# IONIQ6000/av1-base

Hardware: AMD Instinct MI355X
Metric: encoded frames/sec at CQ=30 (1080p intra-only) (higher is better)
Workload: dtype i32; 1 GPU; 1920x1080 60-frame all-key-frame synthclip v1 chunk per GPU, 10-bit 4:2:0, CQ=30 (base_q_idx 120), 32x32 blocks, all 13 intra candidates, 64x64 tiles, adaptive CDFs, CDEF on; frames_per_chunk=60, chunks_per_gpu=1, parallelism=chunk-per-gpu x1

## Files before the change

### av1-base_amd/csrc/av1mi_dev.h

```cpp
#ifndef AV1MI_DEV_H
#define AV1MI_DEV_H
#include <stdint.h>
#include <stddef.h>
#ifdef __HIPCC__
#define AV1MI_HD __host__ __device__
#else
#define AV1MI_HD
#endif

#define AV1MI_QM_4X4 0
#define AV1MI_QM_8X8 16
#define AV1MI_QM_16X16 80
#define AV1MI_QM_32X32 336
#define AV1MI_QM_PLANE 1360

struct Av1miQmEntry { uint32_t q, recip; };

struct Av1miDevParams {
  int width, height, bit_depth;
  int true_w, true_h;
  int mi_rows, mi_cols;
  int sb_rows, sb_cols;
  int tile_sb;
  int tile_rows, tile_cols;
  int b8_rows, b8_cols;
  int n_frames;
  int base_q_idx, qctx;
  int dc_q, ac_q;
  uint32_t dc_recip, ac_recip;
  const Av1miQmEntry *qm_tab;
  int using_qm, qm_y, qm_uv;
// ... 18 lines not shown
  int stream_cap;
  int seq_hdr_bytes, frame_hdr_bytes, inter_hdr_bytes, hdr_slot_bytes;
  int tile_size_bytes;
  int keyint, me_range;
  int subpel;
  int me_presearch;
  int lf_level[4], lf_level_inter[4], lf_sharpness;
  int enable_lr;
  int lr_code_len[4][3];
  unsigned long long lr_code_bits[4][3];
  int sgr_code_len[4][3];
  unsigned long long sgr_code_bits[4][3];
  int lr_chroma;
  int lr_code_len_uv[4][3];
  unsigned long long lr_code_bits_uv[4][3];
};

AV1MI_HD inline int av1mi_node_split(int width, int height, int min_bs_log2, int max_bs_log2, int have_mask, uint32_t mask,
                                     int sb_x, int sb_y, int ox, int oy, int bsl) {
  const int n = 1 << bsl;
  if (bsl <= 3) return 0;
  if (sb_y + oy + (n >> 1) >= height || sb_x + ox + (n >> 1) >= width) return 1;
  if (bsl <= min_bs_log2) return 0;
  if (bsl > max_bs_log2) return 1;
  if (!have_mask) return 0;
  const int bit = bsl == 6 ? 0 : (bsl == 5 ? 1 + ((oy >> 5) << 1 | (ox >> 5))
                                           : 5 + (((ox >> 4) & 1) | (((oy >> 4) & 1) << 1) | (((ox >> 5) & 1) << 2) | (((oy >> 5) & 1) << 3)));
  return (int)((mask >> bit) & 1u);
}
AV1MI_HD inline int av1mi_leaf_bsl_at(int width, int height, int min_bs_log2, int max_bs_log2, int have_mask, uint32_t mask,
// ... 3 lines not shown
    const int ox = bx & ~(n - 1), oy = by & ~(n - 1);
    if (!av1mi_node_split(width, height, min_bs_log2, max_bs_log2, have_mask, mask, sb_x, sb_y, ox, oy, bsl)) return (ox == bx && oy == by) ? bsl : 0;
  }
  return 0;
}

AV1MI_HD inline int av1mi_sext12(uint32_t v) { return (int)((v & 0xFFFu) ^ 0x800u) - 0x800; }
AV1MI_HD inline void av1mi_me_key_decode(unsigned long long key, int R, int *dy, int *dx, int *cost) {
  const int nc = 2 * R + 1, idx = (int)(key & 0xFFFF);
  *dy = idx / nc - R + 8 * av1mi_sext12((uint32_t)(key >> 52));
  *dx = idx % nc - R + 8 * av1mi_sext12((uint32_t)(key >> 40));
  *cost = (int)((key >> 16) & 0xFFFFFF);
}

AV1MI_HD inline int av1mi_frame_is_inter(const Av1miDevParams &P, int f) { return P.keyint > 1 && (f % P.keyint) != 0; }

struct Av1miBlkInfo {
  uint8_t ymode;
  uint8_t skip;
  uint8_t bsl;
  uint8_t is_inter;
  uint16_t eob[3];
  int16_t mv_row, mv_col;
  uint16_t angle;
};
static_assert(sizeof(Av1miBlkInfo) == 16, "block info is one 16-byte record");

#define AV1MI_SB_LEVELS 6144
AV1MI_HD inline int av1mi_morton8(int ux, int uy) {
  return (ux & 1) | ((uy & 1) << 1) | ((ux & 2) << 1) | ((uy & 2) << 2) | ((ux & 4) << 2) | ((uy & 4) << 3);
// ... 54 lines not shown
```

### av1-base_amd/csrc/av1mi_host.cpp

```cpp
#include <hip/hip_runtime.h>
#include <errno.h>
#include <math.h>
#include <stdarg.h>
#include <stdio.h>
#include <stdlib.h>
#include <string.h>
#include <unistd.h>

#include <algorithm>
#include <atomic>
#include <cstddef>
#include <mutex>
#include <string>
#include <thread>
#include <vector>

#include "../../include/av1mi.h"
#include "av1_tables.h"
#include "av1mi_dev.h"

extern "C" {
hipError_t av1mi_launch_partition(const Av1miDevParams *P, const void *frames, uint32_t *part, hipStream_t stream);
#define AV1MI_RECON_PROTO(name) hipError_t name(const Av1miDevParams *P, const Av1miDevParams *dP, const void *src, void *rec, int16_t *levels, \
                                               Av1miBlkInfo *blk, const void *ref, const unsigned long long *me_best, const uint32_t *part, hipStream_t s)
// ... 388 lines not shown

enum ChunkEvent { EV_START, EV_SRC_READY, EV_RECON_DONE, EV_SYM_DONE, EV_ENTROPY_DONE, EV_PACK_DONE, EV_DOWNLOAD_DONE,
                  EV_CDEF_START, EV_CDEF_DONE, EV_GROUPS_JOINED, EV_EDGE_FORK, EV_EDGE_JOIN, EV_COUNT };

struct Workspace {
  size_t cap_frames = 0;
  int scale = 0;
  Resolved res = {};
  void *d_src = nullptr, *d_rec = nullptr, *d_fin = nullptr;
  int16_t *d_levels = nullptr; Av1miBlkInfo *d_blk = nullptr;
  uint8_t *d_slots = nullptr, *d_out = nullptr, *d_hdr = nullptr;
  uint16_t *d_cdf = nullptr;
  Av1miDevParams *d_params = nullptr;
  uint32_t *d_tile_bytes = nullptr, *d_tile_off = nullptr, *d_frame_size = nullptr, *d_payload = nullptr, *d_sym = nullptr;
  uint32_t *d_streams = nullptr, *d_combos = nullptr;
  unsigned long long *d_frame_off = nullptr, *d_sse = nullptr;
  int *d_overflow = nullptr;
  unsigned long long *d_me = nullptr;
  void *d_stage = nullptr;
  void *d_cd = nullptr;
  unsigned long long *d_me_sub = nullptr;
  uint16_t *d_quarter = nullptr;
  uint32_t *d_centre = nullptr;
  uint32_t *d_part = nullptr;
  uint32_t *d_me64 = nullptr;
  Av1miQmEntry *d_qm = nullptr;
  std::vector<Av1miQmEntry> h_qm; int qm_key = -1;
  uint8_t *d_lrc = nullptr;
  unsigned long long *d_lrsse = nullptr;
  unsigned long long *d_cdef_err = nullptr;
  int8_t *d_cdef_idx = nullptr;
  uint8_t *d_cdef_sel = nullptr;
  uint8_t *h_out = nullptr;
  size_t out_cap = 0, me64_bytes = 0, h_out_cap = 0;
  std::vector<std::pair<void *, bool>> owned;
};

template <class T>
hipError_t ws_alloc(Workspace &w, T *&p, size_t bytes, bool host = false) {
  for (auto b = w.owned.begin(); p && b != w.owned.end(); ++b)
    if (b->first == (void *)p) { (void)(b->second ? hipHostFree(p) : hipFree(p)); w.owned.erase(b); break; }
  void *v = nullptr;
  const hipError_t e = host ? hipHostMalloc(&v, bytes, hipHostMallocDefault) : hipMalloc(&v, bytes);
  if (e == hipSuccess) w.owned.emplace_back(v, host);
  p = (T *)v;
  return e;
}

// ... 54 lines not shown
    free_workspace(c);
    const size_t nf = n_frames, slot = (size_t)tile_slot_bytes(r, c->cap_scale);
    for (void **b : { &w.d_src, &w.d_rec, &w.d_fin }) HIPCHK(c, ws_alloc(w, *b, nf * frame_bytes));
    HIPCHK(c, ws_alloc(w, w.d_levels, nf * nsb * AV1MI_SB_LEVELS * sizeof(int16_t)));
    HIPCHK(c, ws_alloc(w, w.d_blk, nf * nb8 * sizeof(Av1miBlkInfo)));
    HIPCHK(c, hipMemsetAsync(w.d_blk, 0, nf * nb8 * sizeof(Av1miBlkInfo), c->stream));
    HIPCHK(c, ws_alloc(w, w.d_slots, nf * ntile * slot * 2));
    w.out_cap = nf * (ntile * (slot + 4) + 256);
    HIPCHK(c, ws_alloc(w, w.d_out, w.out_cap));
    HIPCHK(c, ws_alloc(w, w.d_hdr, 256 + nf * 512));
    HIPCHK(c, ws_alloc(w, w.d_cdf, Av1miCdfLayout::TOTAL * sizeof(uint16_t)));
    HIPCHK(c, ws_alloc(w, w.d_params, sizeof(Av1miDevParams)));
    for (uint32_t **b : { &w.d_tile_bytes, &w.d_tile_off, &w.d_sym, &w.d_combos }) HIPCHK(c, ws_alloc(w, *b, nf * nsb * 4));
    HIPCHK(c, ws_alloc(w, w.d_streams, nf * ntile * (size_t)tile_stream_cap(r, c->cap_scale) * 4));
    for (uint32_t **b : { &w.d_frame_size, &w.d_payload }) HIPCHK(c, ws_alloc(w, *b, nf * 4));
    HIPCHK(c, ws_alloc(w, w.d_frame_off, (nf + 1) * 8));
    HIPCHK(c, ws_alloc(w, w.d_sse, nf * 3 * 8));
    HIPCHK(c, ws_alloc(w, w.d_overflow, 4));
    HIPCHK(c, ws_alloc(w, w.d_me, nf * nb8 * 8));
    w.cap_frames = n_frames; w.scale = c->cap_scale;
  }
  const size_t nf = w.cap_frames;
  if (r.padded && !w.d_stage) HIPCHK(c, ws_alloc(w, w.d_stage, nf * (size_t)p.width * p.height * 3 / 2 * bps));
  if (p.partition_search && !w.d_part) HIPCHK(c, ws_alloc(w, w.d_part, nf * nsb * sizeof(uint32_t)));
  if (p.me_presearch && !w.d_quarter) {
    HIPCHK(c, ws_alloc(w, w.d_quarter, nf * (size_t)(r.cw / 4) * (r.ch / 4) * sizeof(uint16_t)));
    HIPCHK(c, ws_alloc(w, w.d_centre, nf * nsb * sizeof(uint32_t)));
  }
  if (p.subpel && !w.d_me_sub) HIPCHK(c, ws_alloc(w, w.d_me_sub, nf * nb8 * 8));
  if (p.block_log2 >= 6 && p.keyint > 1) {
    const size_t nc = 2 * (size_t)(p.me_range ? p.me_range : 8) + 1, need = nf * nsb * nc * nc * sizeof(uint32_t);
    if (w.me64_bytes < need) { w.me64_bytes = 0; HIPCHK(c, ws_alloc(w, w.d_me64, need)); w.me64_bytes = need; }
  }
// ... 17 lines not shown
      for (int pt = 0; pt < 2; pt++)
        for (int l2 = 2; l2 <= 5; l2++)
          for (int i = 0; i < (1 << (2 * l2)); i++) {
            const uint32_t q = (uint32_t)(i ? r.ac_q : r.dc_q);
            const uint32_t q2 = (q * av1_qm_iwt[r.qm_level][pt][off[l2 - 2] + i] + 16) >> 5;
            w.h_qm[pt * AV1MI_QM_PLANE + off[l2 - 2] + i] = { q2, (uint32_t)((((uint64_t)1 << 32) + q2 - 1) / q2) };
          }
      HIPCHK(c, hipMemcpyAsync(w.d_qm, w.h_qm.data(), w.h_qm.size() * sizeof(Av1miQmEntry), hipMemcpyHostToDevice, c->stream));
      w.qm_key = key;
    }
  }
  return AV1MI_OK;
}

Av1miDevParams dev_params(const Resolved &r, uint32_t n_frames, int scale, const uint32_t *part, const Av1miQmEntry *qm,
                          unsigned long long *cdef_err, int8_t *cdef_idx, uint8_t *cdef_sel) {
  const av1mi_params &p = r.p;
  Av1miDevParams P;
  memset(&P, 0, sizeof(P));
  P.width = r.cw; P.height = r.ch; P.bit_depth = p.bit_depth; P.true_w = (int)p.width; P.true_h = (int)p.height;
  P.mi_rows = r.ch / 4; P.mi_cols = r.cw / 4; P.b8_rows = r.ch / 8; P.b8_cols = r.cw / 8; P.sb_rows = r.sb_rows; P.sb_cols = r.sb_cols;
  P.tile_sb = r.tile_sb; P.tile_rows = r.tile_rows; P.tile_cols = r.tile_cols;
  P.n_frames = (int)n_frames;
  P.base_q_idx = r.qidx;
  P.qctx = r.qidx <= 20 ? 0 : (r.qidx <= 60 ? 1 : (r.qidx <= 120 ? 2 : 3));
  P.dc_q = r.dc_q; P.ac_q = r.ac_q;
  P.dc_recip = (uint32_t)((((uint64_t)1 << 32) + P.dc_q - 1) / P.dc_q);
  P.ac_recip = (uint32_t)((((uint64_t)1 << 32) + P.ac_q - 1) / P.ac_q);
  P.using_qm = p.enable_qm ? 1 : 0; P.qm_y = P.qm_uv = r.qm_level;
  P.qm_tab = p.enable_qm && r.qm_level < 15 ? qm : nullptr;
  P.max_bs_log2 = (int)p.block_log2;
// ... 2 lines not shown
  P.mode_mask = p.intra_mode_mask ? (p.intra_mode_mask & 0x1FFF) : 0x0007;
  P.angle_delta = p.intra_angle_delta ? 1 : 0; P.edge_filter = p.intra_edge_filter ? 1 : 0; P.cfl = p.cfl ? 1 : 0; P.tx_search = p.tx_search ? 1 : 0;
  P.enable_cdef = p.enable_cdef ? 1 : 0;
  P.cdef_y_pri = p.cdef_y_pri; P.cdef_y_sec = p.cdef_y_sec; P.cdef_uv_pri = p.cdef_uv_pri; P.cdef_uv_sec = p.cdef_uv_sec;
  P.cdef_damping = p.cdef_damping; P.cdef_search = (int)p.cdef_search;
  if (p.cdef_search) { P.cdef_bits = (int)p.cdef_search - 1; P.cdef_err = cdef_err; P.cdef_idx = cdef_idx; P.cdef_sel = cdef_sel; }
  P.disable_cdf_update = p.cdf_update ? 0 : 1;
  P.stride_y = r.cw; P.stride_c = r.cw / 2; P.frame_samples = (long)r.cw * r.ch * 3 / 2;
  P.plane_off_u = (long)r.cw * r.ch; P.plane_off_v = P.plane_off_u + (long)(r.cw / 2) * (r.ch / 2);
  P.tile_slot_bytes = tile_slot_bytes(r, scale); P.stream_cap = tile_stream_cap(r, scale); P.tile_size_bytes = 4;
  P.keyint = (int)p.keyint; P.me_range = (int)p.me_range; P.subpel = p.subpel ? 1 : 0; P.me_presearch = p.me_presearch ? 1 : 0;
  P.hdr_slot_bytes = 512;
  for (int i = 0; i < 4; i++) { P.lf_level[i] = deblock_level(r, true); P.lf_level_inter[i] = deblock_level(r, false); }
  P.enable_lr = (int)p.enable_lr;
  P.lr_chroma = r.lr_chroma;
  for (int rf = 0; rf < 4; rf++)
    for (int k = 0; k < 3; k++) {
      const BitString b = lr_code_of(rf, k); P.lr_code_len[rf][k] = b.len; P.lr_code_bits[rf][k] = b.bits;
      const BitString g = sgr_code_of(rf, k); P.sgr_code_len[rf][k] = g.len; P.sgr_code_bits[rf][k] = g.bits;
      const BitString u = lr_code_of_uv(rf, k); P.lr_code_len_uv[rf][k] = u.len; P.lr_code_bits_uv[rf][k] = u.bits;
    }
  return P;
}

}

extern "C" {

uint32_t av1mi_abi_version(void) { return AV1MI_ABI_VERSION; }
uint32_t av1mi_struct_sizes(uint32_t *sizes, uint32_t cap) {
// ... 245 lines not shown
static int prepare_chunk(av1mi_ctx *c, const Resolved &r, const void *frames, uint32_t n_frames, int frames_on_device, const void **d_src) {
  Av1miDevParams &P = c->P; Workspace &w = c->ws; hipStream_t s = c->stream;
  size_t str_key = 0, str_inter = 0;
  std::vector<uint8_t> seq = make_sequence_header(r), fh = make_frame_header(r, nullptr, 0, false, &str_key), fhi = make_frame_header(r, nullptr, 0, true, &str_inter);
  P.cdef_str_bit[0] = (int)str_key; P.cdef_str_bit[1] = (int)str_inter;
  P.seq_hdr_bytes = (int)seq.size(); P.frame_hdr_bytes = (int)fh.size(); P.inter_hdr_bytes = (int)fhi.size();
  if (seq.size() > 256 || fh.size() > (size_t)P.hdr_slot_bytes || fhi.size() > (size_t)P.hdr_slot_bytes) { set_err(c, "internal: header larger than its slot"); return AV1MI_E_OVERFLOW; }
  std::vector<uint8_t> blob(seq.size() + (size_t)n_frames * P.hdr_slot_bytes, 0);
  memcpy(blob.data(), seq.data(), seq.size());
  for (uint32_t f = 0; f < n_frames; f++) {
    const bool inter = av1mi_frame_is_inter(P, (int)f);
    std::vector<uint8_t> &h = inter ? fhi : fh;
    if (r.p.film_grain && f) h = make_frame_header(r, nullptr, f, inter);
    memcpy(blob.data() + seq.size() + (size_t)f * P.hdr_slot_bytes, h.data(), h.size());
  }
  std::vector<uint16_t> cdf = make_cdf_blob(r.qidx);
  HIPCHK(c, hipMemcpyAsync(w.d_hdr, blob.data(), blob.size(), hipMemcpyHostToDevice, s));
  HIPCHK(c, hipMemcpyAsync(w.d_cdf, cdf.data(), cdf.size() * 2, hipMemcpyHostToDevice, s));
  HIPCHK(c, hipMemcpyAsync(w.d_params, &P, sizeof(P), hipMemcpyHostToDevice, s));
  HIPCHK(c, hipMemsetAsync(w.d_overflow, 0, 4, s));
  HIPCHK(c, hipMemsetAsync(w.d_sse, 0, (size_t)n_frames * 24, s));
  if (P.cdef_search) HIPCHK(c, hipMemsetAsync(w.d_cdef_err, 0, (size_t)n_frames * P.sb_rows * P.sb_cols * 24 * sizeof(unsigned long long), s));
  HIPCHK(c, hipEventRecord(c->ev[EV_START], s));
  const size_t bytes = (size_t)n_frames * (r.padded ? (size_t)r.p.width * r.p.height * 3 / 2 : (size_t)P.frame_samples) * (P.bit_depth > 8 ? 2 : 1);
  if (!frames_on_device) HIPCHK(c, hipMemcpyAsync(r.padded ? w.d_stage : w.d_src, frames, bytes, hipMemcpyHostToDevice, s));
  if (r.padded) HIPCHK(c, av1mi_launch_pad(frames_on_device ? frames : w.d_stage, w.d_src, (int)r.p.width, (int)r.p.height, r.cw, r.ch, P.bit_depth, (int)n_frames, 0, s));
  *d_src = frames_on_device && !r.padded ? frames : w.d_src;
  if (P.part_map) HIPCHK(c, av1mi_launch_partition(&P, *d_src, w.d_part, s));
  HIPCHK(c, hipEventRecord(c->ev[EV_SRC_READY], s));
  return AV1MI_OK;
}

static decltype(&av1mi_launch_recon_u8) recon_launcher(const Av1miDevParams &P) {
  return P.max_bs_log2 >= 6 ? (P.bit_depth == 8 ? av1mi_launch_recon64_u8 : av1mi_launch_recon64_u16)
                            : (P.bit_depth == 8 ? av1mi_launch_recon_u8 : av1mi_launch_recon_u16);
// ... 96 lines not shown
      HIPCHK(c, hipEventRecord(c->grp_ev[n_grp], s));
      HIPCHK(c, hipStreamWaitEvent(c->stream3, c->grp_ev[n_grp], 0));
      HIPCHK(c, av1mi_launch_entropy(&P, w.d_cdf, w.d_levels, w.d_blk, w.d_streams, w.d_sym, w.d_combos, w.d_slots, w.d_tile_bytes, w.d_lrc,
                                     w.d_tile_off, (int)(f + 1 - grp), (int)grp, c->stream3, nullptr, nullptr, nullptr, nullptr));
      n_grp++;
    }
  }
  if (n_grp) HIPCHK(c, hipEventRecord(c->ev[EV_GROUPS_JOINED], c->stream3));
  const int rc = entropy_code(c, n_grp * grp, n_frames);
  return rc ? rc : sse_beside_range_coder(c, src);
}

static int download_chunk(av1mi_ctx *c, const Resolved &r, uint32_t n_frames, int frames_on_device, av1mi_buf *out, uint32_t *frame_sizes,
                          void *recon, av1mi_report *report) {
  const Av1miDevParams &P = c->P; Workspace &w = c->ws; hipStream_t s = c->stream, s2 = c->stream2;
  std::vector<unsigned long long> foff(n_frames + 1);
  int overflow = 0;
  HIPCHK(c, hipMemcpyAsync(foff.data(), w.d_frame_off, (n_frames + 1) * 8, hipMemcpyDeviceToHost, s));
  HIPCHK(c, hipMemcpyAsync(&overflow, w.d_overflow, 4, hipMemcpyDeviceToHost, s));
  HIPCHK(c, hipStreamSynchronize(s));
  if (overflow) {
    (void)hipStreamSynchronize(s2);
    set_err(c, "a tile outgrew its %d-byte bitstream slot or its %d-entry symbol stream", P.tile_slot_bytes, P.stream_cap);
    return AV1MI_E_OVERFLOW;
  }
  const size_t total = (size_t)foff[n_frames];
  if (total > w.out_cap) { (void)hipStreamSynchronize(s2); set_err(c, "internal: packed size exceeds buffer"); return AV1MI_E_OVERFLOW; }
  uint8_t *host = (uint8_t *)pin_acquire(total ? total : 1);
  const bool direct = host != nullptr;
  if (!direct) {
    host = (uint8_t *)malloc(total ? total : 1);
    if (!host) { (void)hipStreamSynchronize(s2); return AV1MI_E_OOM; }
    if (w.h_out_cap < total) {
      w.h_out_cap = 0;
      if (ws_alloc(w, w.h_out, total + (total >> 2) + 4096, true) == hipSuccess) w.h_out_cap = total + (total >> 2) + 4096;
    }
  }
  uint8_t *dst = direct ? host : (w.h_out ? w.h_out : host);
  hipError_t e1 = hipMemcpyAsync(dst, w.d_out, total, hipMemcpyDeviceToHost, s);
  hipError_t e2 = hipEventRecord(c->ev[EV_DOWNLOAD_DONE], s);
  if (e2 == hipSuccess) e2 = hipStreamWaitEvent(s, c->ev[EV_CDEF_DONE], 0);
  if (e1 == hipSuccess && e2 == hipSuccess && recon) {
    const void *fin = w.d_fin;
    if (r.padded) {
      e1 = av1mi_launch_pad(w.d_fin, w.d_stage, (int)r.p.width, (int)r.p.height, r.cw, r.ch, P.bit_depth, (int)n_frames, 1, s);
      fin = w.d_stage;
    }
    const size_t bytes = (size_t)n_frames * (r.padded ? (size_t)r.p.width * r.p.height * 3 / 2 : (size_t)P.frame_samples) * (P.bit_depth > 8 ? 2 : 1);
    if (e1 == hipSuccess) e1 = hipMemcpyAsync(recon, fin, bytes, frames_on_device ? hipMemcpyDeviceToDevice : hipMemcpyDeviceToHost, s);
  }
  std::vector<unsigned long long> sse(n_frames * 3);
  std::vector<uint32_t> syms;
  if (e1 == hipSuccess) e1 = hipMemcpyAsync(sse.data(), w.d_sse, (size_t)n_frames * 24, hipMemcpyDeviceToHost, s);
  if (e1 == hipSuccess && report) {
    syms.resize((size_t)n_frames * P.tile_rows * P.tile_cols);
    e1 = hipMemcpyAsync(syms.data(), w.d_sym, syms.size() * 4, hipMemcpyDeviceToHost, s);
  }
  if (e1 == hipSuccess && e2 == hipSuccess) e1 = hipEventSynchronize(c->ev[EV_DOWNLOAD_DONE]);
  if (e1 == hipSuccess && e2 == hipSuccess && dst != host) memcpy(host, dst, total);
  if (e1 == hipSuccess) e1 = hipStreamSynchronize(s);
  if (e1 != hipSuccess || e2 != hipSuccess) {
    (void)hipStreamSynchronize(s2);
    av1mi_free(host);
    set_err(c, "device-to-host copy failed: %s", hipGetErrorString(e1 != hipSuccess ? e1 : e2));
    return AV1MI_E_HIP;
  }
  out->data = host; out->size = total;
  if (frame_sizes) for (uint32_t f = 0; f < n_frames; f++) frame_sizes[f] = (uint32_t)(foff[f + 1] - foff[f]);
  if (report) {
    memset(report, 0, sizeof(*report));
    report->frames = n_frames; report->bytes = total; report->chunks = 1;
    report->cap_scale = (uint32_t)c->cap_scale; report->gpus_used = 1u << (c->device & 31);
    const double mx = (double)((1 << P.bit_depth) - 1);
    for (int pl = 0; pl < 3; pl++) {
      double t = 0;
      for (uint32_t f = 0; f < n_frames; f++) t += (double)sse[f * 3 + pl];
      report->sse[pl] = t;
      const double npx = (double)n_frames * P.width * P.height / (pl ? 4 : 1);
      report->psnr[pl] = t > 0 ? 10.0 * log10(mx * mx * npx / t) : 99.0;
    }
    for (uint32_t v : syms) { report->n_symbols += v; if (v > report->max_tile_symbols) report->max_tile_symbols = v; }
    (void)hipEventElapsedTime(&report->ms_h2d, c->ev[EV_START], c->ev[EV_SRC_READY]);
    (void)hipEventElapsedTime(&report->ms_recon, c->ev[EV_SRC_READY], c->ev[EV_RECON_DONE]);
    (void)hipEventElapsedTime(&report->ms_cdef, c->ev[EV_CDEF_START], c->ev[EV_CDEF_DONE]);
    (void)hipEventElapsedTime(&report->ms_entropy, c->ev[EV_RECON_DONE], c->ev[EV_ENTROPY_DONE]);
    (void)hipEventElapsedTime(&report->ms_symbolize, c->ev[EV_RECON_DONE], c->ev[EV_SYM_DONE]);
    (void)hipEventElapsedTime(&report->ms_pack, c->ev[EV_ENTROPY_DONE], c->ev[EV_PACK_DONE]);
    (void)hipEventElapsedTime(&report->ms_d2h, c->ev[EV_PACK_DONE], c->ev[EV_DOWNLOAD_DONE]);
    (void)hipEventElapsedTime(&report->ms_total, c->ev[EV_START], c->ev[EV_DOWNLOAD_DONE]);
  }
  return AV1MI_OK;
}

static int encode_chunk_once(av1mi_ctx *c, const av1mi_params *params, const void *frames, uint32_t n_frames, int frames_on_device,
                             av1mi_buf *out, uint32_t *frame_sizes, void *recon, av1mi_report *report) {
  out->data = nullptr; out->size = 0;
  Resolved r;
  int rc = resolve(params, &r);
  if (rc) { set_err(c, "invalid parameters"); return rc; }
  HIPCHK(c, hipSetDevice(c->device));
  rc = ensure_workspace(c, r, n_frames);
  if (rc) return rc;
  Workspace &w = c->ws;
  c->P = dev_params(r, n_frames, c->cap_scale, w.d_part, w.d_qm, w.d_cdef_err, w.d_cdef_idx, w.d_cdef_sel);
  const void *d_src = nullptr;
  rc = prepare_chunk(c, r, frames, n_frames, frames_on_device, &d_src);
  if (rc) return rc;
  const Av1miDevParams &P = c->P;
  if (P.keyint > 1 && n_frames > 1) rc = schedule_inter(c, d_src, n_frames);
  else if (P.enable_lr) rc = schedule_all_key_lr(c, d_src, n_frames);
  else rc = schedule_all_key(c, d_src, n_frames);
  if (rc) return rc;
  for (int stage = 0; stage < 2; stage++)
    HIPCHK(c, av1mi_launch_pack(&P, w.d_slots, w.d_tile_bytes, w.d_tile_off, w.d_frame_size, w.d_payload, w.d_frame_off, w.d_hdr,
                                w.d_out, w.d_overflow, stage, c->stream));
  HIPCHK(c, hipEventRecord(c->ev[EV_PACK_DONE], c->stream));
  return download_chunk(c, r, n_frames, frames_on_device, out, frame_sizes, recon, report);
}

}
```

### av1-base_amd/csrc/cdef_pack_kernels.hip

```cpp
#include <hip/hip_runtime.h>
#include "av1mi_dev.h"

namespace {

__constant__ int c_div_table[9] = { 0, 840, 420, 280, 210, 168, 140, 120, 105 };

struct CdefLds {
  uint8_t dir[64];
  uint8_t on[64];
  uint16_t pri_y[64];
};
__shared__ CdefLds g_cdef;

__device__ __forceinline__ int iabs(int v) { return v < 0 ? -v : v; }
__device__ __forceinline__ int constrain(int diff, int threshold, int shift) {
  const int mag = iabs(diff);
  int lim = threshold - (mag >> shift);
  lim = lim < 0 ? 0 : (lim > mag ? mag : lim);
  return diff < 0 ? -lim : lim;
}
__device__ __forceinline__ int damp_shift(int threshold, int damping) {
  if (!threshold) return 0;
  const int a = damping - (31 - __builtin_clz((unsigned)threshold));
  return a < 0 ? 0 : a;
// ... 572 lines not shown
    for (int o = 32; o > 0; o >>= 1) v += __shfl_xor(v, o, 64);
    if ((threadIdx.x & 63) == 0 && v) atomicAdd(&sse[f * 3 + pl], v);
  }
}

__device__ __forceinline__ int leb128_len(uint32_t v) {
  int n = 1;
  while (v >>= 7) n++;
  return n;
}

__global__ void __launch_bounds__(256) frame_layout_kernel(Av1miDevParams P, const uint32_t *__restrict__ tile_bytes,
                                                          uint32_t *__restrict__ tile_off, uint32_t *__restrict__ frame_size,
                                                          uint32_t *__restrict__ payload_size, int *__restrict__ overflow) {
  __shared__ uint32_t part[256];
  const int f = blockIdx.x, nt = P.tile_rows * P.tile_cols, t = threadIdx.x;
  const uint32_t *tb = tile_bytes + (size_t)f * nt;
  const int per = (nt + 255) / 256;
  uint32_t s = 0;
  for (int i = t * per; i < (t + 1) * per && i < nt; i++) {
    if (tb[i] > (uint32_t)P.tile_slot_bytes) atomicExch(overflow, 1);
    s += tb[i] + (i < nt - 1 ? (uint32_t)P.tile_size_bytes : 0u);
  }
  part[t] = s;
  __syncthreads();
  if (t == 0) {
    const int inter = av1mi_frame_is_inter(P, f);
    uint32_t run = (uint32_t)(inter ? P.inter_hdr_bytes : P.frame_hdr_bytes);
    for (int i = 0; i < 256; i++) { uint32_t v = part[i]; part[i] = run; run += v; }
    payload_size[f] = run;
    frame_size[f] = 2u + (inter ? 0u : (uint32_t)P.seq_hdr_bytes) + 1u + (uint32_t)leb128_len(run) + run;
  }
  __syncthreads();
  uint32_t run = part[t];
  for (int i = t * per; i < (t + 1) * per && i < nt; i++) {
    tile_off[(size_t)f * nt + i] = run;
    run += tb[i] + (i < nt - 1 ? (uint32_t)P.tile_size_bytes : 0u);
  }
}

__global__ void chunk_layout_kernel(int n_frames, const uint32_t *__restrict__ frame_size, unsigned long long *__restrict__ frame_off) {
  if (threadIdx.x == 0 && blockIdx.x == 0) {
    unsigned long long run = 0;
    for (int f = 0; f < n_frames; f++) { frame_off[f] = run; run += frame_size[f]; }
    frame_off[n_frames] = run;
  }
// ... 115 lines not shown
```

### av1-base_amd/csrc/entropy_kernel.hip

```cpp
#include <hip/hip_runtime.h>
#include <cstdlib>
#include "av1mi_dev.h"

namespace {

typedef Av1miCdfLayout CL;

#define ENT_RESOLVED(fl6, fh6, ns) (0x80000000u | ((uint32_t)(fl6) << 14) | ((uint32_t)(fh6) << 4) | (uint32_t)(ns))
#define ENT_NARROW(slot, sym) (((uint32_t)(slot) << 2) | (uint32_t)(sym))
#define ENT_LITERAL(bit) ((bit) ? ENT_RESOLVED(256, 0, 0) : ENT_RESOLVED(512, 256, 1))
#define SLOTS_PER_COMBO 63
#define MAX_COMBOS 2

__shared__ uint16_t g_cdf_narrow[CL::INTRA_TOTAL - CL::COEFF_BASE + 64];
__shared__ uint16_t g_full_list[5 * 64];
__shared__ uint16_t g_cdf_inter[CL::TOTAL - CL::INTER_BASE + 64];
struct InterLds {
  int stk_row[10], stk_col[10], stk_w[10];
  uint8_t newmv[256];
};
__shared__ InterLds g_inter;
struct CC {
  enum {
    LEAD = CL::TX_SET1,
// ... 491 lines not shown
  const int o = z - (cls ? (2 << (cls + 2)) : 0);
  const int d = o >> 3, fr = (o >> 1) & 3;
  sym_wide<1>(y, lane, adapt, v < 0, base + CL::MVC_SIGN, 2);
  sym_wide<1>(y, lane, adapt, cls, base + CL::MVC_CLASS, 11);
  if (cls == 0) {
    sym_wide<1>(y, lane, adapt, d, base + CL::MVC_CLASS0, 2);
    sym_wide<1>(y, lane, adapt, fr, base + CL::MVC_CLASS0_FP + d * 5, 4);
  } else {
    for (int i = 0; i < cls; i++) sym_wide<1>(y, lane, adapt, (d >> i) & 1, base + CL::MVC_BITS + i * 3, 2);
    sym_wide<1>(y, lane, adapt, fr, base + CL::MVC_FP, 4);
  }
}

__device__ __forceinline__ int icdf_prob(const Sym &y, int off, int el) { return (el > 0 ? y.cdf[off + el - 1] : 32768) - y.cdf[off + el]; }

__device__ __forceinline__ bool sb_unsplit(const Av1miDevParams &P, int f, int sbr, int sbc) {
  if (!P.part_map || P.min_bs_log2 >= P.max_bs_log2) return true;
  const uint32_t m = P.part_map[((size_t)f * P.sb_rows + sbr) * P.sb_cols + sbc];
  return P.max_bs_log2 >= 6 ? !(m & 1u) : (P.max_bs_log2 == 5 ? !(m & 0x1Eu) : !(m & 0x1FFFE0u));
}

__device__ __forceinline__ bool sb_uniform(const Av1miDevParams &P, int f, int sbr, int sbc) {
  if (!sb_unsplit(P, f, sbr, sbc)) return false;
  const int L = P.max_bs_log2, n = 1 << L;
  if (L <= 3) return true;
  for (int oy = 0; oy < 64; oy += n)
    for (int ox = 0; ox < 64; ox += n) {
      const int x = sbc * 64 + ox, yy = sbr * 64 + oy;
      if (x < P.width && yy < P.height && (yy + (n >> 1) >= P.height || x + (n >> 1) >= P.width)) return false;
    }
  return true;
}

template <bool FULL, bool INTER, int TSB>
__global__ void __launch_bounds__(64) symbolize_tile_kernel(Av1miDevParams P, const uint16_t *__restrict__ cdf_init,
                                                           const int16_t *__restrict__ levels, const Av1miBlkInfo *__restrict__ blk,
                                                           uint32_t *__restrict__ streams, uint32_t *__restrict__ stream_len,
                                                           uint32_t *__restrict__ tile_combos, const uint8_t *__restrict__ lr_choice,
                                                           int tile0 ) {
  const int tiles_per_frame = P.tile_rows * P.tile_cols, sbs_per_frame = P.sb_rows * P.sb_cols;
  const int gt = (int)blockIdx.x + tile0;
  const int f = gt / tiles_per_frame, tile = gt % tiles_per_frame;
  const int tr = tile / P.tile_cols, tc = tile % P.tile_cols;
  const int lane = threadIdx.x;
  {
    bool regular = !P.disable_cdf_update;
    if (regular)
      for (int si = 0; si < TSB * TSB; si++) {
        const int sbr = tr * TSB + si / TSB, sbc = tc * TSB + si % TSB;
        if (sbr < P.sb_rows && sbc < P.sb_cols) regular = regular && sb_uniform(P, f, sbr, sbc);
      }
    if (regular == FULL) return;
  }
  if constexpr (FULL) {
    for (int i = lane; i < CL::COEFF_BASE; i += 64) g_cdfw_full[i] = cdf_init[i];
    if (lane < 18) g_cdfw_full[CL::COEFF_BASE + lane] = 0;
  } else {
    const int l2y = P.max_bs_log2 > 6 ? 6 : P.max_bs_log2, l2c = l2y - 1 > 5 ? 5 : l2y - 1;
    uint16_t *const w = g_cdfw_compact;
    for (int i = lane; i < CC::LEAD; i += 64) w[i] = cdf_init[i];
    for (int i = lane; i < 13 * 8; i += 64)
      w[CC::TXSET + i] = l2y <= 3 ? cdf_init[CL::TX_SET1 + (l2y - 2) * 13 * 8 + i] : ((l2y == 4 && i < 13 * 6) ? cdf_init[CL::TX_SET2 + (l2y - 2) * 13 * 6 + i] : (uint16_t)0);
    for (int i = lane; i < 2 * 39; i += 64) { const int p = i / 39, txs = (p ? l2c : l2y) - 2; w[CC::TXB_SKIP + i] = cdf_init[CL::TXB_SKIP + txs * 39 + i % 39]; }
    if (lane < 24) {
      const int p = lane / 12, k = lane % 12, bwl = (p ? l2c : l2y) > 5 ? 5 : (p ? l2c : l2y), msz = 2 * bwl - 4, nsy = 5 + msz;
      const int eoff = CL::EOB16 + 4 * (msz * 6 + (msz * (msz - 1)) / 2) + (p * 2 + 0) * (nsy + 1);
      w[CC::EOB + lane] = k <= nsy ? cdf_init[eoff + k] : (uint16_t)0;
    }
// ... 555 lines not shown
  if (wave == 1) rc_finish(T, out, tile_bytes);
}

}

extern "C" hipError_t av1mi_launch_entropy(const Av1miDevParams *P, const uint16_t *cdf_init, const int16_t *levels,
                                           const Av1miBlkInfo *blk, uint32_t *streams, uint32_t *stream_len, uint32_t *tile_combos,
                                           uint8_t *slots, uint32_t *tile_bytes, const uint8_t *lr_choice, uint32_t *tile_order ,
                                           int frame0, int count ,
                                           hipStream_t stream, hipEvent_t mid,
                                           hipStream_t aux, hipEvent_t fork, hipEvent_t join ) {
  const int tpf = P->tile_rows * P->tile_cols;
  const int n_tiles = count * tpf, tile0 = frame0 * tpf;
  bool has_inter = false, has_key = false;
  for (int f = frame0; f < frame0 + count; f++) { if (av1mi_frame_is_inter(*P, f)) has_inter = true; else has_key = true; }
  hipStream_t fs = stream;
  if (aux) {
    (void)hipEventRecord(fork, stream);
    (void)hipStreamWaitEvent(aux, fork, 0);
    fs = aux;
  }
#define SYM_LAUNCH(FULLV, INTERV, TSBV)                                                                                                   \
  hipLaunchKernelGGL((symbolize_tile_kernel<FULLV, INTERV, TSBV>), dim3(n_tiles), dim3(64), 0, (FULLV) ? fs : stream, *P, cdf_init, levels, blk, streams, \
                     stream_len, tile_combos, lr_choice, tile0)
  if (P->tile_sb == 1) {
    if (has_key) { SYM_LAUNCH(false, false, 1); SYM_LAUNCH(true, false, 1); }
    if (has_inter) { SYM_LAUNCH(false, true, 1); SYM_LAUNCH(true, true, 1); }
  } else {
    if (has_key) { SYM_LAUNCH(false, false, 2); SYM_LAUNCH(true, false, 2); }
    if (has_inter) { SYM_LAUNCH(false, true, 2); SYM_LAUNCH(true, true, 2); }
  }
#undef SYM_LAUNCH
  if (aux) {
    (void)hipEventRecord(join, aux);
    (void)hipStreamWaitEvent(stream, join, 0);
  }
  if (mid) (void)hipEventRecord(mid, stream);
  const char *const stages_str = getenv("AV1MI_RC_STAGES");
  const int stages_env = stages_str ? atoi(stages_str) : 0;
  const int n_groups = (n_tiles + 63) / 64;
  const int stages = stages_env == 2 || stages_env == 4 ? stages_env : (n_groups <= 256 || n_groups > 512 || (has_inter && P->base_q_idx >= 64) ? 4 : 2);
  bool sorted = n_groups > (stages == 4 ? 256 : 512);
  if (const char *so = getenv("AV1MI_RC_SORT")) sorted = atoi(so) != 0;
  if (sorted) hipLaunchKernelGGL(tile_order_kernel, dim3(1), dim3(1024), 0, stream, n_tiles, stream_len + tile0, tile_order + tile0);
  if (stages == 4)
    hipLaunchKernelGGL(rangecode4_tiles_kernel, dim3(n_groups), dim3(256), 0, stream, *P, n_tiles, cdf_init, streams, stream_len,
                       tile_combos, slots, tile_bytes, sorted ? tile_order + tile0 : (uint32_t *)nullptr, tile0);
  else
// ... 5 lines not shown
```

Baseline: 20530 frames/s.

## Cache host uploads, fold chunk stats on device, shrink irregular symbolize grid

Header, CDF and params uploads are now skipped when their content is unchanged since the previous chunk, using pinned host staging. Symbol counts, overflow and frame offsets are reduced into one device chunk record so a single download replaces several. When no partition map exists, the FULL symbolize kernel launches only over the edge tiles instead of every tile, and launches are skipped when one class is empty. Cached-upload state must be invalidated on errors, and the edge-tile shortcut assumes only edge tiles can be irregular.

Measured after the change: 20940 frames/s (median of 6 runs). +2.0%, better.

```diff
diff --git a/av1-base_amd/csrc/av1mi_dev.h b/av1-base_amd/csrc/av1mi_dev.h
--- a/av1-base_amd/csrc/av1mi_dev.h
+++ b/av1-base_amd/csrc/av1mi_dev.h
@@ -15,6 +15,14 @@
 #define AV1MI_QM_PLANE 1360
 
 struct Av1miQmEntry { uint32_t q, recip; };
+
+struct Av1miChunkRecord {
+  unsigned long long n_symbols;
+  uint32_t max_tile_symbols;
+  int overflow;
+};
+static_assert(sizeof(Av1miChunkRecord) == 16, "the frame offsets follow the head, 8-byte aligned");
+
 
 struct Av1miDevParams {
   int width, height, bit_depth;
@@ -63,6 +71,8 @@
   int lr_chroma;
   int lr_code_len_uv[4][3];
   unsigned long long lr_code_bits_uv[4][3];
+  Av1miChunkRecord *chunk_record;
+  const uint32_t *tile_symbols;
 };
 
 AV1MI_HD inline int av1mi_node_split(int width, int height, int min_bs_log2, int max_bs_log2, int have_mask, uint32_t mask,
@@ -96,6 +106,35 @@
 }
 
 AV1MI_HD inline int av1mi_frame_is_inter(const Av1miDevParams &P, int f) { return P.keyint > 1 && (f % P.keyint) != 0; }
+
+AV1MI_HD inline bool av1mi_sb_unsplit(const Av1miDevParams &P, int f, int sbr, int sbc) {
+  if (!P.part_map || P.min_bs_log2 >= P.max_bs_log2) return true;
+  const uint32_t m = P.part_map[((size_t)f * P.sb_rows + sbr) * P.sb_cols + sbc];
+  return P.max_bs_log2 >= 6 ? !(m & 1u) : (P.max_bs_log2 == 5 ? !(m & 0x1Eu) : !(m & 0x1FFFE0u));
+}
+AV1MI_HD inline bool av1mi_sb_uniform(const Av1miDevParams &P, int f, int sbr, int sbc) {
+  if (!av1mi_sb_unsplit(P, f, sbr, sbc)) return false;
+  const int L = P.max_bs_log2, n = 1 << L;
+  if (L <= 3) return true;
+  for (int oy = 0; oy < 64; oy += n)
+    for (int ox = 0; ox < 64; ox += n) {
+      const int x = sbc * 64 + ox, yy = sbr * 64 + oy;
+      if (x < P.width && yy < P.height && (yy + (n >> 1) >= P.height || x + (n >> 1) >= P.width)) return false;
+    }
+  return true;
+}
+AV1MI_HD inline bool av1mi_tile_is_regular(const Av1miDevParams &P, int f, int tr, int tc, int tsb) {
+  if (P.disable_cdf_update) return false;
+  for (int si = 0; si < tsb * tsb; si++) {
+    const int sbr = tr * tsb + si / tsb, sbc = tc * tsb + si % tsb;
+    if (sbr < P.sb_rows && sbc < P.sb_cols && !av1mi_sb_uniform(P, f, sbr, sbc)) return false;
+  }
+  return true;
+}
+AV1MI_HD inline int av1mi_edge_tiles(const Av1miDevParams &P) { return P.tile_cols + P.tile_rows - 1; }
+AV1MI_HD inline int av1mi_edge_tile(const Av1miDevParams &P, int e) {
+  return e < P.tile_cols ? (P.tile_rows - 1) * P.tile_cols + e : (e - P.tile_cols) * P.tile_cols + P.tile_cols - 1;
+}
 
 struct Av1miBlkInfo {
   uint8_t ymode;
diff --git a/av1-base_amd/csrc/av1mi_host.cpp b/av1-base_amd/csrc/av1mi_host.cpp
--- a/av1-base_amd/csrc/av1mi_host.cpp
+++ b/av1-base_amd/csrc/av1mi_host.cpp
@@ -426,8 +426,8 @@
   Av1miDevParams *d_params = nullptr;
   uint32_t *d_tile_bytes = nullptr, *d_tile_off = nullptr, *d_frame_size = nullptr, *d_payload = nullptr, *d_sym = nullptr;
   uint32_t *d_streams = nullptr, *d_combos = nullptr;
-  unsigned long long *d_frame_off = nullptr, *d_sse = nullptr;
-  int *d_overflow = nullptr;
+  unsigned long long *d_sse = nullptr;
+  Av1miChunkRecord *d_record = nullptr;
   unsigned long long *d_me = nullptr;
   void *d_stage = nullptr;
   void *d_cd = nullptr;
@@ -444,6 +444,11 @@
   int8_t *d_cdef_idx = nullptr;
   uint8_t *d_cdef_sel = nullptr;
   uint8_t *h_out = nullptr;
+  uint8_t *h_hdr = nullptr; uint16_t *h_cdf = nullptr; Av1miDevParams *h_params = nullptr;
+  size_t hdr_bytes = 0;
+  int cdf_qidx = -1;
+  bool params_on_device = false;
+  Av1miChunkRecord *h_record = nullptr; unsigned long long *h_sse = nullptr;
   size_t out_cap = 0, me64_bytes = 0, h_out_cap = 0;
   std::vector<std::pair<void *, bool>> owned;
 };
@@ -528,9 +533,20 @@
     for (uint32_t **b : { &w.d_tile_bytes, &w.d_tile_off, &w.d_sym, &w.d_combos }) HIPCHK(c, ws_alloc(w, *b, nf * nsb * 4));
     HIPCHK(c, ws_alloc(w, w.d_streams, nf * ntile * (size_t)tile_stream_cap(r, c->cap_scale) * 4));
     for (uint32_t **b : { &w.d_frame_size, &w.d_payload }) HIPCHK(c, ws_alloc(w, *b, nf * 4));
-    HIPCHK(c, ws_alloc(w, w.d_frame_off, (nf + 1) * 8));
+    HIPCHK(c, ws_alloc(w, w.d_record, sizeof(Av1miChunkRecord) + (nf + 1) * 8));
     HIPCHK(c, ws_alloc(w, w.d_sse, nf * 3 * 8));
-    HIPCHK(c, ws_alloc(w, w.d_overflow, 4));
+    {
+      auto up = [](size_t n) { return (n + 255) & ~(size_t)255; };
+      const size_t b_hdr = up(256 + nf * 512), b_cdf = up(Av1miCdfLayout::TOTAL * sizeof(uint16_t)), b_par = up(sizeof(Av1miDevParams)),
+                   b_rec = up(sizeof(Av1miChunkRecord) + (nf + 1) * 8), b_sse = up(nf * 3 * 8);
+      uint8_t *h = nullptr;
+      HIPCHK(c, ws_alloc(w, h, b_hdr + b_cdf + b_par + b_rec + b_sse, true));
+      w.h_hdr = h; h += b_hdr;
+      w.h_cdf = reinterpret_cast<uint16_t *>(h); h += b_cdf;
+      w.h_params = reinterpret_cast<Av1miDevParams *>(h); h += b_par;
+      w.h_record = reinterpret_cast<Av1miChunkRecord *>(h); h += b_rec;
+      w.h_sse = reinterpret_cast<unsigned long long *>(h);
+    }
     HIPCHK(c, ws_alloc(w, w.d_me, nf * nb8 * 8));
     w.cap_frames = n_frames; w.scale = c->cap_scale;
   }
@@ -578,7 +594,7 @@
 }
 
 Av1miDevParams dev_params(const Resolved &r, uint32_t n_frames, int scale, const uint32_t *part, const Av1miQmEntry *qm,
-                          unsigned long long *cdef_err, int8_t *cdef_idx, uint8_t *cdef_sel) {
+                          unsigned long long *cdef_err, int8_t *cdef_idx, uint8_t *cdef_sel, Av1miChunkRecord *record, const uint32_t *tile_symbols) {
   const av1mi_params &p = r.p;
   Av1miDevParams P;
   memset(&P, 0, sizeof(P));
@@ -611,6 +627,7 @@
   for (int i = 0; i < 4; i++) { P.lf_level[i] = deblock_level(r, true); P.lf_level_inter[i] = deblock_level(r, false); }
   P.enable_lr = (int)p.enable_lr;
   P.lr_chroma = r.lr_chroma;
+  P.chunk_record = record; P.tile_symbols = tile_symbols;
   for (int rf = 0; rf < 4; rf++)
     for (int k = 0; k < 3; k++) {
       const BitString b = lr_code_of(rf, k); P.lr_code_len[rf][k] = b.len; P.lr_code_bits[rf][k] = b.bits;
@@ -886,11 +903,26 @@
     if (r.p.film_grain && f) h = make_frame_header(r, nullptr, f, inter);
     memcpy(blob.data() + seq.size() + (size_t)f * P.hdr_slot_bytes, h.data(), h.size());
   }
-  std::vector<uint16_t> cdf = make_cdf_blob(r.qidx);
-  HIPCHK(c, hipMemcpyAsync(w.d_hdr, blob.data(), blob.size(), hipMemcpyHostToDevice, s));
-  HIPCHK(c, hipMemcpyAsync(w.d_cdf, cdf.data(), cdf.size() * 2, hipMemcpyHostToDevice, s));
-  HIPCHK(c, hipMemcpyAsync(w.d_params, &P, sizeof(P), hipMemcpyHostToDevice, s));
-  HIPCHK(c, hipMemsetAsync(w.d_overflow, 0, 4, s));
+  if (w.hdr_bytes != blob.size() || memcmp(w.h_hdr, blob.data(), blob.size())) {
+    w.hdr_bytes = 0;
+    memcpy(w.h_hdr, blob.data(), blob.size());
+    HIPCHK(c, hipMemcpyAsync(w.d_hdr, w.h_hdr, blob.size(), hipMemcpyHostToDevice, s));
+  }
+  w.hdr_bytes = P.cdef_search ? 0 : blob.size();
+  if (w.cdf_qidx != r.qidx) {
+    w.cdf_qidx = -1;
+    const std::vector<uint16_t> cdf = make_cdf_blob(r.qidx);
+    memcpy(w.h_cdf, cdf.data(), cdf.size() * 2);
+    HIPCHK(c, hipMemcpyAsync(w.d_cdf, w.h_cdf, cdf.size() * 2, hipMemcpyHostToDevice, s));
+    w.cdf_qidx = r.qidx;
+  }
+  if (!w.params_on_device || memcmp(w.h_params, &P, sizeof(P))) {
+    w.params_on_device = false;
+    memcpy(w.h_params, &P, sizeof(P));
+    HIPCHK(c, hipMemcpyAsync(w.d_params, w.h_params, sizeof(P), hipMemcpyHostToDevice, s));
+    w.params_on_device = true;
+  }
+  HIPCHK(c, hipMemsetAsync(w.d_record, 0, sizeof(Av1miChunkRecord), s));
   HIPCHK(c, hipMemsetAsync(w.d_sse, 0, (size_t)n_frames * 24, s));
   if (P.cdef_search) HIPCHK(c, hipMemsetAsync(w.d_cdef_err, 0, (size_t)n_frames * P.sb_rows * P.sb_cols * 24 * sizeof(unsigned long long), s));
   HIPCHK(c, hipEventRecord(c->ev[EV_START], s));
@@ -1017,30 +1049,34 @@
 static int download_chunk(av1mi_ctx *c, const Resolved &r, uint32_t n_frames, int frames_on_device, av1mi_buf *out, uint32_t *frame_sizes,
                           void *recon, av1mi_report *report) {
   const Av1miDevParams &P = c->P; Workspace &w = c->ws; hipStream_t s = c->stream, s2 = c->stream2;
-  std::vector<unsigned long long> foff(n_frames + 1);
-  int overflow = 0;
-  HIPCHK(c, hipMemcpyAsync(foff.data(), w.d_frame_off, (n_frames + 1) * 8, hipMemcpyDeviceToHost, s));
-  HIPCHK(c, hipMemcpyAsync(&overflow, w.d_overflow, 4, hipMemcpyDeviceToHost, s));
-  HIPCHK(c, hipStreamSynchronize(s));
-  if (overflow) {
+  const Av1miChunkRecord &rec = *w.h_record;
+  const unsigned long long *foff = reinterpret_cast<const unsigned long long *>(w.h_record + 1);
+  hipError_t e1 = hipMemcpyAsync(w.h_record, w.d_record, sizeof(Av1miChunkRecord) + (n_frames + 1) * 8, hipMemcpyDeviceToHost, s);
+  if (e1 == hipSuccess) e1 = hipStreamSynchronize(s);
+  if (e1 != hipSuccess) {
     (void)hipStreamSynchronize(s2);
-    set_err(c, "a tile outgrew its %d-byte bitstream slot or its %d-entry symbol stream", P.tile_slot_bytes, P.stream_cap);
+    set_err(c, "fetching the chunk record failed: %s", hipGetErrorString(e1));
+    return AV1MI_E_HIP;
+  }
+  if (rec.overflow || foff[n_frames] > w.out_cap) {
+    (void)hipStreamSynchronize(s2);
+    if (rec.overflow) set_err(c, "a tile outgrew its %d-byte bitstream slot or its %d-entry symbol stream", P.tile_slot_bytes, P.stream_cap);
+    else set_err(c, "internal: packed size exceeds buffer");
     return AV1MI_E_OVERFLOW;
   }
   const size_t total = (size_t)foff[n_frames];
-  if (total > w.out_cap) { (void)hipStreamSynchronize(s2); set_err(c, "internal: packed size exceeds buffer"); return AV1MI_E_OVERFLOW; }
-  uint8_t *host = (uint8_t *)pin_acquire(total ? total : 1);
-  const bool direct = host != nullptr;
-  if (!direct) {
+  uint8_t *host = (uint8_t *)pin_acquire(total ? total : 1), *dst = host;
+  if (!host) {
     host = (uint8_t *)malloc(total ? total : 1);
     if (!host) { (void)hipStreamSynchronize(s2); return AV1MI_E_OOM; }
     if (w.h_out_cap < total) {
       w.h_out_cap = 0;
       if (ws_alloc(w, w.h_out, total + (total >> 2) + 4096, true) == hipSuccess) w.h_out_cap = total + (total >> 2) + 4096;
     }
-  }
-  uint8_t *dst = direct ? host : (w.h_out ? w.h_out : host);
-  hipError_t e1 = hipMemcpyAsync(dst, w.d_out, total, hipMemcpyDeviceToHost, s);
+    if (w.h_out && w.h_out_cap >= total) dst = w.h_out;
+    else dst = host;
+  }
+  e1 = hipMemcpyAsync(dst, w.d_out, total, hipMemcpyDeviceToHost, s);
   hipError_t e2 = hipEventRecord(c->ev[EV_DOWNLOAD_DONE], s);
   if (e2 == hipSuccess) e2 = hipStreamWaitEvent(s, c->ev[EV_CDEF_DONE], 0);
   if (e1 == hipSuccess && e2 == hipSuccess && recon) {
@@ -1052,15 +1088,12 @@
     const size_t bytes = (size_t)n_frames * (r.padded ? (size_t)r.p.width * r.p.height * 3 / 2 : (size_t)P.frame_samples) * (P.bit_depth > 8 ? 2 : 1);
     if (e1 == hipSuccess) e1 = hipMemcpyAsync(recon, fin, bytes, frames_on_device ? hipMemcpyDeviceToDevice : hipMemcpyDeviceToHost, s);
   }
-  std::vector<unsigned long long> sse(n_frames * 3);
-  std::vector<uint32_t> syms;
-  if (e1 == hipSuccess) e1 = hipMemcpyAsync(sse.data(), w.d_sse, (size_t)n_frames * 24, hipMemcpyDeviceToHost, s);
-  if (e1 == hipSuccess && report) {
-    syms.resize((size_t)n_frames * P.tile_rows * P.tile_cols);
-    e1 = hipMemcpyAsync(syms.data(), w.d_sym, syms.size() * 4, hipMemcpyDeviceToHost, s);
-  }
-  if (e1 == hipSuccess && e2 == hipSuccess) e1 = hipEventSynchronize(c->ev[EV_DOWNLOAD_DONE]);
-  if (e1 == hipSuccess && e2 == hipSuccess && dst != host) memcpy(host, dst, total);
+  const unsigned long long *sse = w.h_sse;
+  if (e1 == hipSuccess) e1 = hipMemcpyAsync(w.h_sse, w.d_sse, (size_t)n_frames * 24, hipMemcpyDeviceToHost, s);
+  if (e1 == hipSuccess && e2 == hipSuccess && dst != host) {
+    e1 = hipEventSynchronize(c->ev[EV_DOWNLOAD_DONE]);
+    if (e1 == hipSuccess) memcpy(host, dst, total);
+  }
   if (e1 == hipSuccess) e1 = hipStreamSynchronize(s);
   if (e1 != hipSuccess || e2 != hipSuccess) {
     (void)hipStreamSynchronize(s2);
@@ -1082,7 +1115,7 @@
       const double npx = (double)n_frames * P.width * P.height / (pl ? 4 : 1);
       report->psnr[pl] = t > 0 ? 10.0 * log10(mx * mx * npx / t) : 99.0;
     }
-    for (uint32_t v : syms) { report->n_symbols += v; if (v > report->max_tile_symbols) report->max_tile_symbols = v; }
+    report->n_symbols = rec.n_symbols; report->max_tile_symbols = rec.max_tile_symbols;
     (void)hipEventElapsedTime(&report->ms_h2d, c->ev[EV_START], c->ev[EV_SRC_READY]);
     (void)hipEventElapsedTime(&report->ms_recon, c->ev[EV_SRC_READY], c->ev[EV_RECON_DONE]);
     (void)hipEventElapsedTime(&report->ms_cdef, c->ev[EV_CDEF_START], c->ev[EV_CDEF_DONE]);
@@ -1095,8 +1128,21 @@
   return AV1MI_OK;
 }
 
+static int run_chunk(av1mi_ctx *c, const av1mi_params *params, const void *frames, uint32_t n_frames, int frames_on_device,
+                     av1mi_buf *out, uint32_t *frame_sizes, void *recon, av1mi_report *report);
+
 static int encode_chunk_once(av1mi_ctx *c, const av1mi_params *params, const void *frames, uint32_t n_frames, int frames_on_device,
                              av1mi_buf *out, uint32_t *frame_sizes, void *recon, av1mi_report *report) {
+  const int rc = run_chunk(c, params, frames, n_frames, frames_on_device, out, frame_sizes, recon, report);
+  if (rc != AV1MI_OK && rc != AV1MI_E_OVERFLOW) {
+    (void)hipStreamSynchronize(c->stream);
+    c->ws.hdr_bytes = 0; c->ws.cdf_qidx = -1; c->ws.params_on_device = false;
+  }
+  return rc;
+}
+
+static int run_chunk(av1mi_ctx *c, const av1mi_params *params, const void *frames, uint32_t n_frames, int frames_on_device,
+                     av1mi_buf *out, uint32_t *frame_sizes, void *recon, av1mi_report *report) {
   out->data = nullptr; out->size = 0;
   Resolved r;
   int rc = resolve(params, &r);
@@ -1105,7 +1151,7 @@
   rc = ensure_workspace(c, r, n_frames);
   if (rc) return rc;
   Workspace &w = c->ws;
-  c->P = dev_params(r, n_frames, c->cap_scale, w.d_part, w.d_qm, w.d_cdef_err, w.d_cdef_idx, w.d_cdef_sel);
+  c->P = dev_params(r, n_frames, c->cap_scale, w.d_part, w.d_qm, w.d_cdef_err, w.d_cdef_idx, w.d_cdef_sel, w.d_record, w.d_sym);
   const void *d_src = nullptr;
   rc = prepare_chunk(c, r, frames, n_frames, frames_on_device, &d_src);
   if (rc) return rc;
@@ -1115,8 +1161,8 @@
   else rc = schedule_all_key(c, d_src, n_frames);
   if (rc) return rc;
   for (int stage = 0; stage < 2; stage++)
-    HIPCHK(c, av1mi_launch_pack(&P, w.d_slots, w.d_tile_bytes, w.d_tile_off, w.d_frame_size, w.d_payload, w.d_frame_off, w.d_hdr,
-                                w.d_out, w.d_overflow, stage, c->stream));
+    HIPCHK(c, av1mi_launch_pack(&P, w.d_slots, w.d_tile_bytes, w.d_tile_off, w.d_frame_size, w.d_payload,
+                                reinterpret_cast<unsigned long long *>(w.d_record + 1), w.d_hdr, w.d_out, &w.d_record->overflow, stage, c->stream));
   HIPCHK(c, hipEventRecord(c->ev[EV_PACK_DONE], c->stream));
   return download_chunk(c, r, n_frames, frames_on_device, out, frame_sizes, recon, report);
 }
diff --git a/av1-base_amd/csrc/cdef_pack_kernels.hip b/av1-base_amd/csrc/cdef_pack_kernels.hip
--- a/av1-base_amd/csrc/cdef_pack_kernels.hip
+++ b/av1-base_amd/csrc/cdef_pack_kernels.hip
@@ -610,10 +610,19 @@
                                                           uint32_t *__restrict__ tile_off, uint32_t *__restrict__ frame_size,
                                                           uint32_t *__restrict__ payload_size, int *__restrict__ overflow) {
   __shared__ uint32_t part[256];
+  __shared__ unsigned long long sym_sum[256];
+  __shared__ uint32_t sym_max[256];
   const int f = blockIdx.x, nt = P.tile_rows * P.tile_cols, t = threadIdx.x;
   const uint32_t *tb = tile_bytes + (size_t)f * nt;
   const int per = (nt + 255) / 256;
   uint32_t s = 0;
+  if (P.chunk_record) {
+    const uint32_t *sl = P.tile_symbols + (size_t)f * nt;
+    unsigned long long ssum = 0;
+    uint32_t smax = 0;
+    for (int i = t * per; i < (t + 1) * per && i < nt; i++) { ssum += sl[i]; smax = sl[i] > smax ? sl[i] : smax; }
+    sym_sum[t] = ssum; sym_max[t] = smax;
+  }
   for (int i = t * per; i < (t + 1) * per && i < nt; i++) {
     if (tb[i] > (uint32_t)P.tile_slot_bytes) atomicExch(overflow, 1);
     s += tb[i] + (i < nt - 1 ? (uint32_t)P.tile_size_bytes : 0u);
@@ -626,6 +635,13 @@
     for (int i = 0; i < 256; i++) { uint32_t v = part[i]; part[i] = run; run += v; }
     payload_size[f] = run;
     frame_size[f] = 2u + (inter ? 0u : (uint32_t)P.seq_hdr_bytes) + 1u + (uint32_t)leb128_len(run) + run;
+    if (P.chunk_record) {
+      unsigned long long ssum = 0;
+      uint32_t smax = 0;
+      for (int i = 0; i < 256; i++) { ssum += sym_sum[i]; smax = sym_max[i] > smax ? sym_max[i] : smax; }
+      atomicAdd(&P.chunk_record->n_symbols, ssum);
+      atomicMax(&P.chunk_record->max_tile_symbols, smax);
+    }
   }
   __syncthreads();
   uint32_t run = part[t];
diff --git a/av1-base_amd/csrc/entropy_kernel.hip b/av1-base_amd/csrc/entropy_kernel.hip
--- a/av1-base_amd/csrc/entropy_kernel.hip
+++ b/av1-base_amd/csrc/entropy_kernel.hip
@@ -529,44 +529,20 @@
 
 __device__ __forceinline__ int icdf_prob(const Sym &y, int off, int el) { return (el > 0 ? y.cdf[off + el - 1] : 32768) - y.cdf[off + el]; }
 
-__device__ __forceinline__ bool sb_unsplit(const Av1miDevParams &P, int f, int sbr, int sbc) {
-  if (!P.part_map || P.min_bs_log2 >= P.max_bs_log2) return true;
-  const uint32_t m = P.part_map[((size_t)f * P.sb_rows + sbr) * P.sb_cols + sbc];
-  return P.max_bs_log2 >= 6 ? !(m & 1u) : (P.max_bs_log2 == 5 ? !(m & 0x1Eu) : !(m & 0x1FFFE0u));
-}
-
-__device__ __forceinline__ bool sb_uniform(const Av1miDevParams &P, int f, int sbr, int sbc) {
-  if (!sb_unsplit(P, f, sbr, sbc)) return false;
-  const int L = P.max_bs_log2, n = 1 << L;
-  if (L <= 3) return true;
-  for (int oy = 0; oy < 64; oy += n)
-    for (int ox = 0; ox < 64; ox += n) {
-      const int x = sbc * 64 + ox, yy = sbr * 64 + oy;
-      if (x < P.width && yy < P.height && (yy + (n >> 1) >= P.height || x + (n >> 1) >= P.width)) return false;
-    }
-  return true;
-}
-
 template <bool FULL, bool INTER, int TSB>
 __global__ void __launch_bounds__(64) symbolize_tile_kernel(Av1miDevParams P, const uint16_t *__restrict__ cdf_init,
                                                            const int16_t *__restrict__ levels, const Av1miBlkInfo *__restrict__ blk,
                                                            uint32_t *__restrict__ streams, uint32_t *__restrict__ stream_len,
                                                            uint32_t *__restrict__ tile_combos, const uint8_t *__restrict__ lr_choice,
-                                                           int tile0 ) {
+                                                           int tile0 ,
+                                                           int edge_grid ) {
   const int tiles_per_frame = P.tile_rows * P.tile_cols, sbs_per_frame = P.sb_rows * P.sb_cols;
-  const int gt = (int)blockIdx.x + tile0;
+  int gt = (int)blockIdx.x + tile0;
+  if (edge_grid) { const int ne = av1mi_edge_tiles(P); gt = (tile0 / tiles_per_frame + (int)blockIdx.x / ne) * tiles_per_frame + av1mi_edge_tile(P, (int)blockIdx.x % ne); }
   const int f = gt / tiles_per_frame, tile = gt % tiles_per_frame;
   const int tr = tile / P.tile_cols, tc = tile % P.tile_cols;
   const int lane = threadIdx.x;
-  {
-    bool regular = !P.disable_cdf_update;
-    if (regular)
-      for (int si = 0; si < TSB * TSB; si++) {
-        const int sbr = tr * TSB + si / TSB, sbc = tc * TSB + si % TSB;
-        if (sbr < P.sb_rows && sbc < P.sb_cols) regular = regular && sb_uniform(P, f, sbr, sbc);
-      }
-    if (regular == FULL) return;
-  }
+  if (av1mi_tile_is_regular(P, f, tr, tc, TSB) == FULL) return;
   if constexpr (FULL) {
     for (int i = lane; i < CL::COEFF_BASE; i += 64) g_cdfw_full[i] = cdf_init[i];
     if (lane < 18) g_cdfw_full[CL::COEFF_BASE + lane] = 0;
@@ -1152,15 +1128,36 @@
   const int n_tiles = count * tpf, tile0 = frame0 * tpf;
   bool has_inter = false, has_key = false;
   for (int f = frame0; f < frame0 + count; f++) { if (av1mi_frame_is_inter(*P, f)) has_inter = true; else has_key = true; }
+  bool regular_any = true, full_any = true, edge_grid = false;
+  if (!P->part_map) {
+    regular_any = !P->disable_cdf_update;
+    if (regular_any) {
+      full_any = false;
+      for (int e = 0; e < av1mi_edge_tiles(*P); e++) {
+        const int t = av1mi_edge_tile(*P, e);
+        if (!av1mi_tile_is_regular(*P, 0, t / P->tile_cols, t % P->tile_cols, P->tile_sb)) full_any = true;
+      }
+      edge_grid = full_any;
+    }
+  }
   hipStream_t fs = stream;
-  if (aux) {
+  const bool forked = aux && regular_any && full_any;
+  if (!forked && aux) {
+    (void)hipEventRecord(fork, stream); (void)hipStreamWaitEvent(aux, fork, 0);
+    (void)hipEventRecord(join, aux); (void)hipStreamWaitEvent(stream, join, 0);
+  }
+  if (forked) {
     (void)hipEventRecord(fork, stream);
     (void)hipStreamWaitEvent(aux, fork, 0);
     fs = aux;
   }
+  const int full_grid = edge_grid ? count * av1mi_edge_tiles(*P) : n_tiles;
 #define SYM_LAUNCH(FULLV, INTERV, TSBV)                                                                                                   \
-  hipLaunchKernelGGL((symbolize_tile_kernel<FULLV, INTERV, TSBV>), dim3(n_tiles), dim3(64), 0, (FULLV) ? fs : stream, *P, cdf_init, levels, blk, streams, \
-                     stream_len, tile_combos, lr_choice, tile0)
+  do {                                                                                                                                    \
+    if ((FULLV) ? full_any : regular_any)                                                                                                 \
+      hipLaunchKernelGGL((symbolize_tile_kernel<FULLV, INTERV, TSBV>), dim3((FULLV) ? full_grid : n_tiles), dim3(64), 0, (FULLV) ? fs : stream, *P, cdf_init, \
+                         levels, blk, streams, stream_len, tile_combos, lr_choice, tile0, (FULLV) && edge_grid ? 1 : 0);                  \
+  } while (0)
   if (P->tile_sb == 1) {
     if (has_key) { SYM_LAUNCH(false, false, 1); SYM_LAUNCH(true, false, 1); }
     if (has_inter) { SYM_LAUNCH(false, true, 1); SYM_LAUNCH(true, true, 1); }
@@ -1169,7 +1166,7 @@
     if (has_inter) { SYM_LAUNCH(false, true, 2); SYM_LAUNCH(true, true, 2); }
   }
 #undef SYM_LAUNCH
-  if (aux) {
+  if (forked) {
     (void)hipEventRecord(join, aux);
     (void)hipStreamWaitEvent(stream, join, 0);
   }
```
